# li-kunyi/CUT3R-SLAM

Measured on AMD Instinct MI355X. Metric: frames/sec (ViT pointmap + covisibility-graph tracking step) on 640x480, higher is better.
Workload: dtype f16

## Files before the change

cut3r_slam_amd/_lib.py:

```python
from __future__ import annotations

import ctypes as C
import os

_HERE = os.path.dirname(os.path.abspath(__file__))
LIB_PATH = os.path.join(_HERE, "libcut3r_hip.so")

c_void_p, c_int, c_float, c_ll = C.c_void_p, C.c_int, C.c_float, C.c_longlong


class GemmDesc(C.Structure):
    _fields_ = [
        ("A", c_void_p), ("B", c_void_p), ("C", c_void_p), ("bias", c_void_p), ("res1", c_void_p), ("res2", c_void_p),
        ("M", c_int), ("N", c_int), ("K", c_int), ("lda", c_int), ("ldb", c_int), ("ldc", c_int), ("ldr1", c_int),
        ("ldr2", c_int),
        ("act", c_int), ("out_f16", c_int), ("res1_f16", c_int), ("res2_f16", c_int),
        ("batch", c_int),
        ("strideA", c_ll), ("strideB", c_ll), ("strideC", c_ll), ("strideBias", c_ll), ("strideR1", c_ll),
        ("strideR2", c_ll),
        ("conv_k", c_int), ("H", c_int), ("W", c_int), ("Cin", c_int), ("conv_stride", c_int), ("Ho", c_int),
        ("Wo", c_int), ("relu_in", c_int),
        ("shuf", c_int), ("shuf_cout", c_int), ("shuf_Hin", c_int), ("shuf_Win", c_int),
        ("tile", c_int), ("stages", c_int),
        ("rope_pos", c_void_p), ("rope_table", c_void_p), ("rope_cols", c_int), ("rope_pmin", c_int), ("rope_npos", c_int),
# ... 4 lines not shown


class LcTerm(C.Structure):
    _fields_ = [("a", c_void_p), ("c", c_void_p), ("mask", c_void_p), ("ia", c_int), ("ic", c_int), ("w", c_float), ("pad", c_int)]


SIGNATURES = {
    "cut3r_abi_version": [],
    "cut3r_rope2d": [c_void_p, c_int, c_void_p, c_int, c_int, c_int, c_int, c_ll, c_ll, c_ll, c_float, c_float, c_void_p],
    "cut3r_rope2d_qk": [c_void_p, c_void_p, c_int, c_void_p, c_int, c_int, c_int, c_int, c_ll, c_ll, c_ll, c_ll, c_float, c_float,
                        c_void_p],
    "cut3r_rope2d_tab": [c_void_p, c_void_p, c_ll, c_ll, c_void_p, c_void_p, c_ll, c_ll, c_int, c_int, c_void_p, c_int, c_int, c_float,
                         c_float, c_void_p],
    "cut3r_layernorm": [c_void_p, c_int, c_void_p, c_void_p, c_float, c_int, c_int, c_void_p, c_int, c_void_p, c_int,
                        c_void_p, c_void_p, c_void_p],
    "cut3r_layernorm_dual": [c_void_p, c_int, c_void_p, c_void_p, c_void_p, c_int, c_void_p, c_void_p, c_void_p, c_int, c_float, c_int,
                             c_int, c_void_p],
    "cut3r_gemm_f16": [C.POINTER(GemmDesc), c_void_p],
    "cut3r_gemm_tile_for": [C.POINTER(GemmDesc)],
    "cut3r_gemm_f16_pair": [C.POINTER(GemmDesc), C.POINTER(GemmDesc), c_void_p],
    "cut3r_gemm_kernel_for": [C.POINTER(GemmDesc)],
    "cut3r_gemm_pair_kernel_for": [C.POINTER(GemmDesc), C.POINTER(GemmDesc)],
    "cut3r_gemm_kernel_count": [],
    "cut3r_rope2d_table": [c_void_p, c_int, c_int, c_int, c_float, c_float, c_void_p],
    "cut3r_gemv_f16w": [c_void_p, c_int, c_void_p, c_int, c_void_p, c_void_p, c_int, c_int, c_int, c_int, c_int,
                        c_void_p, c_int, c_int, c_void_p],
    "cut3r_attention_variant": [c_int],
    "cut3r_attention_kernel_for": [c_int, c_int, c_int, c_int],
    "cut3r_attention_f16": [c_void_p, c_void_p, c_void_p, c_void_p, c_int, c_int, c_int, c_int, c_int,
                            c_ll, c_ll, c_ll, c_ll, c_ll, c_ll, c_ll, c_ll, c_float, c_void_p],
    "cut3r_im2col_patch": [c_void_p, c_int, c_int, c_int, c_int, c_int, c_int, c_void_p, c_void_p],
    "cut3r_cast_f32_f16": [c_void_p, c_int, c_void_p, c_int, c_int, c_int, c_void_p],
    "cut3r_colmean": [c_void_p, c_int, c_int, c_int, c_void_p, c_void_p],
    "cut3r_colmean_batched": [c_void_p, c_int, c_ll, c_int, c_int, c_int, c_void_p, c_ll, c_void_p],
    "cut3r_upsample2x_nhwc": [c_void_p, c_void_p, c_int, c_int, c_int, c_int, c_void_p],
    "cut3r_dpt_final": [c_void_p, c_int, c_int, c_void_p, c_void_p, c_int, c_void_p, c_void_p, c_void_p],
    "cut3r_conv3x3_dpt_final": [C.POINTER(GemmDesc), c_void_p, c_void_p, c_int, c_void_p, c_ll, c_void_p, c_ll, c_void_p],
    "cut3r_postprocess_pts": [c_void_p, c_int, c_int, c_int, c_void_p, c_void_p, c_void_p],
    "cut3r_postprocess_pose": [c_void_p, c_int, c_void_p, c_void_p],
    "cut3r_patch_overlap": [c_void_p, c_void_p, c_int, c_int, c_float, c_void_p, c_void_p, c_void_p],
    "cut3r_patch_overlap_chain": [c_void_p, c_void_p, c_int, c_int, c_int, c_float, C.c_double, c_void_p, c_void_p, c_void_p, c_void_p,
                                  c_void_p, c_void_p],
    "cut3r_overlap_fwd": [c_void_p, c_int, C.POINTER(c_float), c_float, c_void_p, c_int, c_float, c_float, c_float, c_float,
                          c_int, c_int, c_int, c_void_p, c_void_p],
    "cut3r_overlap_bwd": [c_void_p, c_int, c_int, c_int, c_int, c_void_p, c_float, c_float, c_float, c_float, c_int, c_int,
                          c_void_p, c_void_p],
# ... 171 lines not shown
```

cut3r_slam_amd/csrc/gemm.hip:

```cpp
#include <cstdlib>
#include "common.h"
#include "dpt_tail.h"
#include "../../include/cut3r_hip.h"

namespace {

constexpr int BK = 64;
constexpr int KCH = BK / 8;

struct GemmArgs {
    const h16* A; const h16* B; void* C;
    const float* bias; const void* res1; const void* res2;
    int M, N, K, lda, ldb, ldc, ldr1, ldr2;
    int act, out_f16, res1_f16, res2_f16;
    long long sA, sB, sC, sBias, sR1, sR2;
    int conv_k, H, W, Cin, cstride, Ho, Wo, relu_in;
    int shuf, shuf_cout, shuf_Hin, shuf_Win;
    int swz;
    int prio;
    const long long* rope_pos; const float* rope_table; int rope_cols, rope_pmin, rope_npos, rope_d;
    const float* ln_stats; const float* ln_c; int ln_nslab; float ln_eps;
    float* stats_out; h16* out16; int ld16;
    const float* dpt_w; const float* dpt_b; float* dpt_pts; float* dpt_conf; long long dpt_pts_vs, dpt_conf_vs;
};
// ... 582 lines not shown
#define CUT3R_TILE_BOUNDS __launch_bounds__(64 * WAVES_M * WAVES_N, (WAVES_M * WAVES_N == 8 && (BM + BN) * BK * 2 * NSTAGE <= 81920) ? 4 : 1)
template <int BM, int BN, int NSTAGE, int WAVES_M = 2, int WAVES_N = 2, int ADDR = 0, int EPI = 0>
__global__ CUT3R_TILE_BOUNDS void gemm_kernel(const GemmArgs g) {
    gemm_tile_body<BM, BN, NSTAGE, WAVES_M, WAVES_N, ADDR, EPI>(g, blockIdx.x, blockIdx.y, blockIdx.z);
}

static int tile_addr_mode(const GemmArgs& g) {
    static const bool off = [] { const char* e = getenv("CUT3R_GEMM_FASTADDR"); return e && atoi(e) == 0; }();
    if (off || (g.K % BK) != 0) return 0;
    if (g.conv_k == 3) return (g.Cin >= 64 && (g.Cin & (g.Cin - 1)) == 0 && g.K == 9 * g.Cin) ? 2 : 0;
    return 1;
}

struct GemmPairArgs { GemmArgs p[2]; int nblk0; };
template <int BM, int BN, int NSTAGE, int WAVES_M = 2, int WAVES_N = 2, int ADDR = 0, int EPI = 0>
__global__ CUT3R_TILE_BOUNDS void gemm_pair_kernel(const GemmPairArgs a) {
    const int sel = (int)blockIdx.x >= a.nblk0 ? 1 : 0;
    gemm_tile_body<BM, BN, NSTAGE, WAVES_M, WAVES_N, ADDR, EPI>(a.p[sel], blockIdx.x - sel * a.nblk0, 0, 0);
}

#ifndef EPI_UNROLL
#define EPI_UNROLL 1
#endif
template <bool CONV3, bool RELU_IN, bool FAST_DMA = false, int EPI = 0, bool LN = false>
DEVINL void gemm256_body(const GemmArgs& g, const int bx, const int bz) {
    constexpr int UNIT = 128 * BK * 2;
    constexpr int BUF = 4 * UNIT;
    static_assert(!LN || EPI == 1 || EPI == 2 || EPI == 6, "the LayerNorm fold feeds the fp16-output epilogues");
    __shared__ __attribute__((aligned(16))) unsigned char smem[2 * BUF + (LN ? 2 * 1024 : 0)];

    const int tid = threadIdx.x, lane = tid & 63, wave = tid >> 6;
    const int wr = wave >> 2, wc = wave & 3;
    const int z = bz;
    const h16* __restrict__ A = g.A + (size_t)z * g.sA;
    const h16* __restrict__ Bm = g.B + (size_t)z * g.sB;
    const int M = g.M, N = g.N, K = g.K;
    int pid_m, pid_n;
    xcd_tile(bx, (M + 255) / 256, (N + 255) / 256, pid_m, pid_n);
    const int m0 = pid_m * 256, n0 = pid_n * 256;
    const h16* zero = reinterpret_cast<const h16*>(g_zero16);

    const int lrow = lane >> 3;
    const int csrc = (lane & 7) ^ lrow;
    const h16* a_ptr[2][2];
    int a_oy[2][2], a_ox[2][2];
    bool a_ok[2][2];
    const h16* b_ptr[2][2];
    bool b_ok[2][2];
#pragma unroll
    for (int q = 0; q < 2; q++)
#pragma unroll
// ... 25 lines not shown
    unsigned a_msk[2][2];
    const int cin_shift = 31 - __builtin_clz((unsigned)(g.Cin > 0 ? g.Cin : 1));
    if (FAST_DMA && CONV3) {
#pragma unroll
        for (int q = 0; q < 2; q++)
#pragma unroll
            for (int i = 0; i < 2; i++) {
                a_pc[q][i] = a_ptr[q][i] + ((ptrdiff_t)a_oy[q][i] * g.W + a_ox[q][i]) * g.Cin + csrc * 8;
                unsigned mk = 0;
#pragma unroll
                for (int t = 0; t < 9; t++) {
                    const int iy = a_oy[q][i] + t / 3, ix = a_ox[q][i] + t % 3;
                    if (a_ok[q][i] && iy >= 0 && iy < g.H && ix >= 0 && ix < g.W) mk |= 1u << t;
                }
                a_msk[q][i] = mk;
            }
    }
#pragma unroll
    for (int q = 0; q < 2; q++)
#pragma unroll
        for (int i = 0; i < 2; i++) {
            const int u = (wave + 8 * i) * 8 + lrow;
            const int gm = min(m0 + (u >> 6) * 128 + q * 64 + (u & 63), M - 1);
            const int gn = min(n0 + (u >> 5) * 64 + q * 32 + (u & 31), N - 1);
            a_off[q][i] = (unsigned)(((size_t)gm * g.lda + csrc * 8) * 2);
            b_off[q][i] = (unsigned)(((size_t)gn * g.ldb + csrc * 8) * 2);
        }
    auto issue_fast = [&](const h16* mat, const unsigned (&off)[2], int kt, int unit) {
        const char* base = reinterpret_cast<const char*>(mat) + (size_t)kt * (BK * 2);
        unsigned char* slot = smem + (kt & 1) * BUF + unit * UNIT;
        const int wave_s = __builtin_amdgcn_readfirstlane(wave);
#pragma unroll
        for (int i = 0; i < 2; i++)
            __builtin_amdgcn_global_load_lds((const __attribute__((address_space(1))) void*)(base + off[i]),
                                             (__attribute__((address_space(3))) void*)(slot + (wave_s + 8 * i) * 1024), 16, 0, 0);
    };
    auto issue_a = [&](int q, int kt, int unit) {
        if (kt >= nt) return;
        if constexpr (fast_dma && !CONV3) { issue_fast(A, a_off[q], kt, unit); return; }
        if constexpr (fast_dma && CONV3) {
            const int k0 = kt * BK;
            const int tap = k0 >> cin_shift;
            const int dy = (tap >= 3) + (tap >= 6), dx = tap - 3 * dy;
            const int delta = (dy * g.W + dx) * g.Cin + (k0 & (g.Cin - 1));
            unsigned char* slot = smem + (kt & 1) * BUF + unit * UNIT;
            const int wave_s = __builtin_amdgcn_readfirstlane(wave);
#pragma unroll
            for (int i = 0; i < 2; i++) {
// ... 148 lines not shown
        CUT3R_QUADRANT(0, 2, fb1);
        CUT3R_BARRIER();
        read_a(buf + 3 * UNIT);
        issue_a(0, t + 2, 0);
        CUT3R_BARRIER();
        CUT3R_QUADRANT(4, 2, fb1);
        CUT3R_BARRIER();
        issue_b(0, t + 2, 1);
        if (t + 2 < nt) wait_vmcnt<4>(); else wait_vmcnt<0>();
        CUT3R_BARRIER();
        CUT3R_QUADRANT(4, 0, fb0);
        CUT3R_BARRIER();
    }
#endif
    if (wr == 0) CUT3R_BARRIER();
#undef CUT3R_QUADRANT

    constexpr int CP = 68;
    float* cs = reinterpret_cast<float*>(smem + wave * 16384);
    const float* bias = g.bias ? g.bias + (size_t)z * g.sBias : nullptr;
    const bool plain = !g.shuf && g.rope_cols == 0;
    const f32x4 zero4 = {0.f, 0.f, 0.f, 0.f};
    const float* lnp = reinterpret_cast<const float*>(smem + 2 * BUF) + wr * 256;
    if constexpr (EPI == 1 || EPI == 2 || EPI == 4 || EPI == 5 || EPI == 6) {
        const int er = lane >> 3, ec = (lane & 7) * 8;
        const int gn = n0 + wc * 64 + ec;
        const bool col_ok = gn + 8 <= N;
        const int gnc = col_ok ? gn : 0;
        const f32x4 b0 = *reinterpret_cast<const f32x4*>(bias + gnc), b1 = *reinterpret_cast<const f32x4*>(bias + gnc + 4);
        f32x4 lc0 = zero4, lc1 = zero4, lpc0 = zero4, lpc1 = zero4;
        if constexpr (LN) { lc0 = *reinterpret_cast<const f32x4*>(g.ln_c + gnc); lc1 = *reinterpret_cast<const f32x4*>(g.ln_c + gnc + 4); }
        const bool rope_here = EPI == 6 && (n0 + wc * 64) < g.rope_cols && col_ok;
        f32x4 pb0 = zero4, pb1 = zero4;
        if (rope_here) {
            const int pc = gnc + ((ec & 16) ? -16 : 16);
            pb0 = *reinterpret_cast<const f32x4*>(bias + pc);
            pb1 = *reinterpret_cast<const f32x4*>(bias + pc + 4);
            if constexpr (LN) { lpc0 = *reinterpret_cast<const f32x4*>(g.ln_c + pc); lpc1 = *reinterpret_cast<const f32x4*>(g.ln_c + pc + 4); }
        }
        constexpr int ROPE_LDS = 48;
        float* tl = cs + 32 * CP;
        int* psl = reinterpret_cast<int*>(tl + ROPE_LDS * 32);
        if (EPI == 6 && __builtin_amdgcn_readfirstlane((n0 + wc * 64) < g.rope_cols)) {
#pragma unroll
            for (int f0 = 0; f0 < ROPE_LDS * 8; f0 += 64) {
                const int f = f0 + lane, p = f >> 3, part = f & 7;
                f32x4 v = zero4;
// ... 696 lines not shown
    g.prio = 0;
    p.k = {gemm_kernel<192, 128, 2, 4, 2, 2, 7>, 512, tile_code(1, 192, 128, 2, 4, 2, 2, 7)};
    p.grid = tile_grid(g.M, g.N, 192, 128, true, 1);
    return CUT3R_OK;
}

extern "C" int cut3r_conv3x3_dpt_final(const cut3r_gemm_desc* d, const float* w, const float* b, int mode, float* pts, long long pts_view_stride,
                                       float* conf, long long conf_view_stride, void* stream) {
    if (!d || mode != 0) return CUT3R_ERR_ARG;
    cut3r_gemm_desc dd = *d;
    dd.C = const_cast<void*>(d->A);
    GemmArgs g;
    Plan<TileFn> p;
    int rc = fill_args(&dd, g);
    if (rc != CUT3R_OK) return rc;
    g.C = nullptr;
    g.dpt_w = w; g.dpt_b = b; g.dpt_pts = pts; g.dpt_conf = conf; g.dpt_pts_vs = pts_view_stride; g.dpt_conf_vs = conf_view_stride;
    rc = plan_dpt_final(&dd, g, p);
    if (rc != CUT3R_OK) return rc;
    hipLaunchKernelGGL(p.k.fn, p.grid, dim3(p.k.block), 0, (hipStream_t)stream, g);
    return cut3r_check_launch();
}

static int select_pair(const cut3r_gemm_desc* d0, const cut3r_gemm_desc* d1, GemmPairArgs& a, Plan<PairFn>& p) {
    if (!d0 || !d1) return CUT3R_ERR_ARG;
    int rc = fill_args(d0, a.p[0]);
    if (rc == CUT3R_OK) rc = fill_args(d1, a.p[1]);
    return rc == CUT3R_OK ? plan_pair(d0, d1, a, p) : rc;
}
extern "C" int cut3r_gemm_pair_kernel_for(const cut3r_gemm_desc* d0, const cut3r_gemm_desc* d1) {
    GemmPairArgs a;
    Plan<PairFn> p;
    return select_pair(d0, d1, a, p) == CUT3R_OK ? p.k.code : 0;
}

extern "C" int cut3r_gemm_f16_pair(const cut3r_gemm_desc* d0, const cut3r_gemm_desc* d1, void* stream) {
    GemmPairArgs a;
    Plan<PairFn> p;
    const int rc = select_pair(d0, d1, a, p);
    if (rc != CUT3R_OK) return rc;
    hipLaunchKernelGGL(p.k.fn, p.grid, dim3(p.k.block), 0, (hipStream_t)stream, a);
    return cut3r_check_launch();
}

extern "C" int cut3r_gemv_f16w(const float* X, int ldx, const void* W, int ldw, const float* bias, float* Y, int ldy, int M,
                               int N, int K, int act, const float* res, int ldr, int silu_in, void* stream) {
// ... 7 lines not shown
```

cut3r_slam_amd/model.py:

```python
from __future__ import annotations

import gc
import math
import os
import re
from dataclasses import dataclass, field
from typing import Dict, List, NamedTuple, Optional

import torch

from . import ops
from .config import Cut3rConfig, production_config, state_dict_schema

F16, F32 = torch.float16, torch.float32


def _env_flag(name: str, default: bool) -> bool:
    return os.environ.get(name, "1" if default else "0") != "0"


def _env_int(name: str, default: int) -> int:
    return int(os.environ.get(name, str(default)))


# ... 61 lines not shown


class Cut3rModel:
    def __init__(self, cfg: Cut3rConfig, state_dict: Dict[str, torch.Tensor], device="cuda:0", minimal: bool = False):
        self.cfg = cfg
        self.device = torch.device(device)
        self.minimal = minimal
        schema = state_dict_schema(cfg)
        missing = [k for k in schema if k not in state_dict]
        if missing:
            raise KeyError(f"state_dict is missing {len(missing)} tensors, e.g. {missing[:4]}")
        for k, shp in schema.items():
            if tuple(state_dict[k].shape) != tuple(shp):
                raise ValueError(f"{k}: shape {tuple(state_dict[k].shape)} != schema {tuple(shp)}")
        self._buf: Dict[tuple, torch.Tensor] = {}
        self._graphs: Dict[tuple, tuple] = {}
        self.use_graphs = _env_flag("CUT3R_GRAPHS", True)
        self.dual_stream = _env_flag("CUT3R_DUAL_STREAM", True)
        self.dual_ln = _env_flag("CUT3R_DUAL_LN", True)
        self.pair_gemm = _env_flag("CUT3R_PAIR_GEMM", False)
        self.pair_rows = _env_int("CUT3R_PAIR_ROWS", 0)
        self.fused_rope = _env_int("CUT3R_FUSED_ROPE", 1)
        self.rope48_rows = _env_int("CUT3R_ROPE48_ROWS", 0)
        self.head_overlap = _env_flag("CUT3R_HEAD_OVERLAP", True)
        self.dpt_fuse = _env_flag("CUT3R_DPT_FUSE", True)
        self.head_chunk = max(1, _env_int("CUT3R_HEAD_CHUNK", 28))
        self.ln_fold = _env_int("CUT3R_LN_FOLD", 1)
        self._head_stream = None
        self._side = None
        self._head_side = None
        self._prep(state_dict)

    @classmethod
    def from_state_dict(cls, cfg, sd, device="cuda:0", **kw):
        return cls(cfg, sd, device, **kw)

    @classmethod
    def from_pretrained(cls, path: str, config: Optional[Cut3rConfig] = None, device="cuda:0", **kw):
        import argparse
        if not os.path.isfile(path):
            raise FileNotFoundError(f"{path}: no checkpoint (this runtime never fetches from a hub)")
        with torch.serialization.safe_globals([argparse.Namespace]):
            ckpt = torch.load(path, map_location="cpu", weights_only=True)
        sd = ckpt["model"] if "model" in ckpt else ckpt
        sd = {(k[7:] if k.startswith("module.") else k): v for k, v in sd.items()}
        if not any(k.startswith("dec_blocks_state") for k in sd):
# ... 125 lines not shown
            c1(q + ".out_conv")
            for u in ("resConfUnit1", "resConfUnit2"):
                c3(f"{q}.{u}.conv1"); c3(f"{q}.{u}.conv2")
        c3(p + ".head.0"); c3(p + ".head.2")
        self.w[p + ".head.4.w"] = sd[p + ".head.4.weight"].reshape(nch, -1).to(device=dev, dtype=F32).contiguous()
        self.w[p + ".head.4.b"] = sd[p + ".head.4.bias"].to(device=dev, dtype=F32).contiguous()

    def buf(self, name, shape, dtype):
        key = (name, tuple(shape), dtype)
        t = self._buf.get(key)
        if t is None:
            t = torch.empty(shape, dtype=dtype, device=self.device)
            self._buf[key] = t
        return t

    def _panel(self, name, rope=None, ln=None):
        L = self.w[name + "@ln"] if ln is not None else self.w[name]
        if rope is not None:
            rope = (rope[0], rope[1], self.cfg.rope_freq, rope[2])
        if ln is not None:
            ln = (ln, L.c, self.cfg.ln_eps)
        return L, rope, ln

    def _linear(self, x16, name, out, act=0, res1=None, res2=None, skinny=False, rope=None, ln=None, emit=None):
        L, rope, ln = self._panel(name, rope, ln)
        return ops.linear(x16, L.w, out, L.b, act, res1, res2, tile=16 if skinny else 0, rope=rope, ln=ln, emit=emit)

    def _project(self, probs, act=0):
        if len(probs) == 1:
            return self._linear(act=act, **probs[0])

        def prob(x16, name, out, res1=None, skinny=False, rope=None, ln=None, emit=None):
            assert not skinny, "the pair kernels have no one-row-per-sequence form"
            L, rope, ln = self._panel(name, rope, ln)
            return (x16, L.w, out, L.b, res1, dict(rope=rope, ln=ln, emit=emit))
        ops.linear_pair(prob(**probs[0]), prob(**probs[1]), act)

    def _folded(self, name):
        return self.ln_fold and (name + "@ln") in self.w

    def _xs(self, tag, x):
        M, Cc = x.shape
        return self.buf(tag + ".x16", (M, Cc), F16), self.buf(tag + ".xst", (Cc // 64, M, 2), F32)

    def _fuse_rope(self, pos, D, rows):
        dims = (64, 48) if (self.fused_rope == 2 or (self.fused_rope and rows <= self.rope48_rows)) else (64,)
        return self.fused_rope and pos is not None and D in dims and pos.is_contiguous() and pos.numel() == 2 * rows

    def _ln(self, x, name, out16=None, out32=None, mod=None):
        g, b = self.w[name]
        ops.layernorm(x, g, b, self.cfg.ln_eps, out16, out32, mod[0] if mod else None, mod[1] if mod else None)

    def _rope(self, t, pos):
        ops.rope_2d_pair(t, pos, None, None, self.cfg.rope_freq, 1.0)

    def _self_attn(self, tag, x_ln16, B, N, heads, pos, p, out, res, ln=None, emit=None):
        Cc = x_ln16.shape[1]
        D = Cc // heads
        sk = N == 1
        qkv = self.buf(tag + ".qkv", (B * N, 3 * Cc), F16)
        fuse = (not sk) and self._fuse_rope(pos, D, B * N)
        self._linear(x_ln16, p + ".qkv", qkv, skinny=sk, rope=(pos, 2 * Cc, D) if fuse else None, ln=ln)
        v5 = qkv.view(B, N, 3, heads, D)
        q, k, v = v5[:, :, 0], v5[:, :, 1], v5[:, :, 2]
        if pos is not None and not fuse:
            ops.rope_2d_pair(q, pos, k, pos, self.cfg.rope_freq, 1.0)
        a = self.buf(tag + ".attn", (B, N, heads, D), F16)
        ops.attention(q, k, v, a, D ** -0.5)
        self._linear(a.view(B * N, Cc), p + ".proj", out, res1=res, skinny=sk, emit=emit)

# ... 94 lines not shown
        s.fold_y = fresh and can(y, Ny, ".cross_attn.projkv")
        s.fold_o = can(out, Nx, ".mlp.fc1")
        s.emit = (out.st, out.x16) if s.fold_o else None
        s.ln16 = self.buf(tag + ".ln16", (B * Nx, C), F16)
        s.y16 = self.buf(tag + ".y16", (B * Ny, C), F16)
        s.qkv = self.buf(tag + ".qkv", (B * Nx, 3 * C), F16)
        s.attn = self.buf(tag + ".attn", (B, Nx, heads, D), F16)
        s.q = self.buf(tag + ".q", (B, Nx, heads, D), F16)
        s.kv = self.buf(tag + ".kv", (B * Ny, 2 * C), F16)
        s.cattn = self.buf(tag + ".cattn", (B, Nx, heads, D), F16)
        s.mlp_h = self.buf(tag + ".mlp_h", (B * Nx, self.w[p + ".mlp.fc1"].npad), F16)
        return s

    def _pair_carries(self, rows):
        return rows <= self.pair_rows

    def _dec_layer(self, blocks, fork=False):
        pair = len(blocks) == 2
        assert not pair or all(s.Nx > 1 and s.Ny > 1 for s in blocks), "pair launches need more than one row per sequence"
        carry = pair and self._pair_carries(max(s.B * max(s.Nx, s.Ny) for s in blocks))
        assert not pair or carry or not any(s.fold_x or s.fold_y or s.fold_o for s in blocks), "the plain pair kernels take no LayerNorm fold"
        fuse = lambda s, pos, n: bool(n > 1 and self._fuse_rope(pos, s.D, s.B * n) and (not pair or (carry and s.D == 64)))
        fuse_x, fuse_y = (lambda s: fuse(s, s.xpos, s.Nx)), (lambda s: fuse(s, s.ypos, s.Ny))

        def each(fn, need=lambda s: True):
            todo = [s for s in blocks if need(s)]
            if fork and len(todo) == 2:
                cur = torch.cuda.current_stream()
                self._side.wait_stream(cur)
                with torch.cuda.stream(self._side):
                    fn(todo[0])
                fn(todo[1])
                cur.wait_stream(self._side)
            else:
                for s in todo:
                    fn(s)

        rows = lambda t: t.view(-1, t.shape[-2] * t.shape[-1])
        skx, sky = (lambda s: s.Nx == 1), (lambda s: s.Ny == 1)
        each(lambda s: self._ln(s.x.x, s.p + ".norm1", out16=s.ln16), lambda s: not (s.fold_x or s.pre_ln))
        self._project([dict(x16=s.x.x16 if s.fold_x else s.ln16, name=s.p + ".attn.qkv", out=s.qkv, skinny=skx(s),
                            rope=(s.xpos, 2 * s.C, s.D) if fuse_x(s) else None, ln=s.x.st if s.fold_x else None) for s in blocks])

        def self_attn(s):
            v5 = s.qkv.view(s.B, s.Nx, 3, s.heads, s.D)
            q, k, v = v5[:, :, 0], v5[:, :, 1], v5[:, :, 2]
            if s.xpos is not None and not fuse_x(s):
                ops.rope_2d_pair(q, s.xpos, k, s.xpos, self.cfg.rope_freq, 1.0)
            ops.attention(q, k, v, s.attn, s.D ** -0.5)
        each(self_attn)
        self._project([dict(x16=rows(s.attn), name=s.p + ".attn.proj", out=s.out.x, res1=s.x.x, skinny=skx(s), emit=s.emit) for s in blocks])
        each(lambda s: self._ln(s.out.x, s.p + ".norm2", out16=s.ln16), lambda s: not s.fold_o)
        self._project([dict(x16=s.out.x16 if s.fold_o else s.ln16, name=s.p + ".cross_attn.projq", out=rows(s.q), skinny=skx(s),
                            rope=(s.xpos, s.C, s.D) if fuse_x(s) else None, ln=s.out.st if s.fold_o else None) for s in blocks])
        rope_q = lambda s: s.xpos is not None and not fuse_x(s)
        norm_y = lambda s: not (s.fold_y or s.pre_ln)

        def q_rope_and_norm_y(s):
            if rope_q(s):
                self._rope(s.q, s.xpos)
            if norm_y(s):
                self._ln(s.y.x, s.p + ".norm_y", out16=s.y16)
        each(q_rope_and_norm_y, lambda s: rope_q(s) or norm_y(s))
        self._project([dict(x16=s.y.x16 if s.fold_y else s.y16, name=s.p + ".cross_attn.projkv", out=s.kv, skinny=sky(s),
                            rope=(s.ypos, s.C, s.D) if fuse_y(s) else None, ln=s.y.st if s.fold_y else None) for s in blocks])

        def cross_attn(s):
            kv4 = s.kv.view(s.B, s.Ny, 2, s.heads, s.D)
            k, v = kv4[:, :, 0], kv4[:, :, 1]
            if s.ypos is not None and not fuse_y(s):
                self._rope(k, s.ypos)
            ops.attention(s.q, k, v, s.cattn, s.D ** -0.5)
        each(cross_attn)
        self._project([dict(x16=rows(s.cattn), name=s.p + ".cross_attn.proj", out=s.out.x, res1=s.out.x, skinny=skx(s), emit=s.emit) for s in blocks])
        each(lambda s: self._ln(s.out.x, s.p + ".norm3", out16=s.ln16), lambda s: not s.fold_o)
        self._project([dict(x16=s.out.x16 if s.fold_o else s.ln16, name=s.p + ".mlp.fc1", out=s.mlp_h, skinny=skx(s),
                            ln=s.out.st if s.fold_o else None) for s in blocks], act=1)
        self._project([dict(x16=s.mlp_h, name=s.p + ".mlp.fc2", out=s.out.x, res1=s.out.x, skinny=skx(s), emit=s.emit) for s in blocks])

    def _dual_norms(self, l, a, s_a):
        pi, ps = f"dec_blocks.{l}", f"dec_blocks_state.{l}"
        Ci = a.shape[1]
        ops.layernorm_dual(a, *self.w[pi + ".norm1"], self.buf("deci.ln16", (a.shape[0], Ci), F16),
                           *self.w[ps + ".norm_y"], self.buf("decs.y16", (a.shape[0], Ci), F16), self.cfg.ln_eps)
        ops.layernorm_dual(s_a, *self.w[ps + ".norm1"], self.buf("decs.ln16", (s_a.shape[0], Ci), F16),
                           *self.w[pi + ".norm_y"], self.buf("deci.y16", (s_a.shape[0], Ci), F16), self.cfg.ln_eps)

    def _mem_inquire(self, gfeat16, mem, B=1):
        cfg = self.cfg
        D = cfg.dec_embed_dim
        x = self.buf("memr.x", (B, 2 * D), F32)
        self._linear(gfeat16, "pose_retriever.proj_q", x[:, :D], skinny=True)
        x[:, D:] = self.masked_token
# ... 407 lines not shown
```

cut3r_slam_amd/ops.py:

```python
from __future__ import annotations

import ctypes as C
import os
from typing import Optional

import torch

from . import _lib, views
from ._lib import GemmDesc, check

F16, F32 = torch.float16, torch.float32


def _stream():
    return C.c_void_p(torch.cuda.current_stream().cuda_stream)


def _p(t: Optional[torch.Tensor]):
    return C.c_void_p(t.data_ptr()) if t is not None else C.c_void_p(0)


def _req(cond, msg):
    if not cond:
        raise ValueError(msg)
# ... 205 lines not shown
    if emit is not None:
        so, o16 = emit
        _cuda(so, o16)
        _req(N % 64 == 0 and so.dtype == F32 and so.is_contiguous() and so.numel() == M * (N // 64) * 2, f"stats_out fp32 [N/64={N // 64}, M={M}, 2]")
        _req(o16.dtype == F16 and o16.shape == (M, N) and o16.stride(1) == 1, "out16 fp16 [M,N]")
        _req(out.dtype == F32 and res1 is not None and res1.dtype == F32 and res2 is None and act == 0 and tile != 16, "emit: fp32 output with an fp32 residual")
        d.stats_out, d.out16, d.ld16 = so.data_ptr(), o16.data_ptr(), o16.stride(0)
    return d


def linear(A, W, out, bias=None, act=0, res1=None, res2=None, tile=0, rope=None, ln=None, emit=None):
    if tile == 16 and A.dim() == 2 and A.shape[0] > 64:
        M = A.shape[0]
        _linear_desc(A, W, out, bias, act, res1, tile, rope, res2=res2)
        for m0 in range(0, M, 64):
            sl = slice(m0, min(M, m0 + 64))
            linear(A[sl], W, out[sl], bias, act, None if res1 is None else res1[sl], None if res2 is None else res2[sl], tile=16)
        return out
    d = _linear_desc(A, W, out, bias, act, res1, tile, rope, ln, emit, res2=res2)
    _launch(d, f"cut3r_gemm_f16 M={d.M} N={d.N} K={d.K}")
    return out


def linear_pair(p0, p1, act=0, tile=0):
    x0 = p0[5] if len(p0) > 5 and p0[5] else {}
    x1 = p1[5] if len(p1) > 5 and p1[5] else {}
    d0 = _linear_desc(p0[0], p0[1], p0[2], p0[3], act, p0[4], tile, pair=True, **x0)
    d1 = _linear_desc(p1[0], p1[1], p1[2], p1[3], act, p1[4], tile, pair=True, **x1)
    _req(d0.N == d1.N and d0.K == d1.K, "pair: same N and K")
    lib = _lib.load()
    check(lib.cut3r_gemm_f16_pair(C.byref(d0), C.byref(d1), _stream()), f"cut3r_gemm_f16_pair M={d0.M}+{d1.M} N={d0.N} K={d0.K}")


def linear_batched(A, W, out, bias=None, act=0, res1=None, tile=0):
    _cuda(A, W, out, bias, res1)
    _req(A.dtype == F16 and W.dtype == F16 and A.dim() == 3 and W.dim() == 3 and out.dim() == 3, "3-D fp16 operands")
    Z, M, K = A.shape
    N = W.shape[1]
    _req(W.shape == (Z, N, K) and out.shape == (Z, M, N), "batched shapes")
    _req(A.stride(2) == 1 and W.stride(2) == 1 and out.stride(2) == 1, "unit inner strides")
    d = GemmDesc()
    _fill_common(d, A, W, out, bias, None, None, act, tile)
    if bias is not None:
        _req(bias.dtype == F32 and bias.shape == (Z, N) and bias.stride(1) == 1, "bias [Z,N]")
        d.strideBias = bias.stride(0)
    if res1 is not None:
# ... 1197 lines not shown
```

include/cut3r_hip.h:

```cpp
#ifndef CUT3R_HIP_H
#define CUT3R_HIP_H
#include <stdint.h>
#ifdef __cplusplus
extern "C" {
#endif

int cut3r_abi_version(void);

int cut3r_rope2d(void* tokens, int dtype, const int64_t* positions, int B, int N, int H, int D,
                 long long sB, long long sN, long long sH, float base, float fwd, void* stream);
int cut3r_rope2d_qk(void* q, void* k, int dtype, const int64_t* positions, int B, int N, int H, int D, long long q_sB,
                    long long q_sN, long long k_sB, long long k_sN, float base, float fwd, void* stream);

int cut3r_rope2d_tab(void* t0, const int64_t* pos0, long long ntok0, long long stride0, void* t1, const int64_t* pos1, long long ntok1,
                     long long stride1, int H, int D, const float* table, int pmin, int npos, float base, float fwd, void* stream);

int cut3r_layernorm(const float* x, int ldx, const float* gamma, const float* beta, float eps, int M, int C,
                    void* y16, int ld16, float* y32, int ld32, const float* mod_scale, const float* mod_shift,
                    void* stream);
int cut3r_layernorm_dual(const float* x, int ldx, const float* g1, const float* b1, void* y1, int ld1, const float* g2,
                         const float* b2, void* y2, int ld2, float eps, int M, int C, void* stream);

typedef struct cut3r_gemm_desc {
    const void* A;
// ... 13 lines not shown
    int shuf;
    int shuf_cout, shuf_Hin, shuf_Win;
    int tile;
    int stages;
    const void* rope_pos;
    const float* rope_table;
    int rope_cols, rope_pmin, rope_npos;
    int rope_d;
    const float* ln_stats;
    const float* ln_colsum;
    int ln_nslab;
    float ln_eps;
    float* stats_out;
    void* out16;
    int ld16;
} cut3r_gemm_desc;
int cut3r_gemm_f16(const cut3r_gemm_desc* d, void* stream);
int cut3r_rope2d_table(float* table, int pmin, int npos, int Q, float base, float fwd, void* stream);
int cut3r_gemm_tile_for(const cut3r_gemm_desc* d);
int cut3r_gemm_f16_pair(const cut3r_gemm_desc* d0, const cut3r_gemm_desc* d1, void* stream);
int cut3r_gemm_kernel_for(const cut3r_gemm_desc* d);
int cut3r_gemm_pair_kernel_for(const cut3r_gemm_desc* d0, const cut3r_gemm_desc* d1);
int cut3r_gemm_kernel_count(void);

int cut3r_gemv_f16w(const float* X, int ldx, const void* W, int ldw, const float* bias, float* Y, int ldy,
                    int M, int N, int K, int act, const float* res, int ldr, int silu_in, void* stream);

int cut3r_attention_f16(const void* q, const void* k, const void* v, void* out, int B, int H, int Nq, int Nk, int D,
                        long long q_sb, long long q_sn, long long k_sb, long long k_sn, long long v_sb, long long v_sn,
                        long long o_sb, long long o_sn, float scale, void* stream);

int cut3r_attention_variant(int v);
int cut3r_attention_kernel_for(int B, int H, int Nq, int D);

int cut3r_im2col_patch(const void* img, int u8, int B, int C, int H, int W, int P, void* out, void* stream);
int cut3r_cast_f32_f16(const float* x, int ldx, void* y, int ldy, int M, int C, void* stream);
int cut3r_colmean(const float* x, int ldx, int M, int C, float* y, void* stream);
int cut3r_colmean_batched(const float* x, int B, long long stride_x, int ldx, int M, int C, float* y, long long stride_y, void* stream);

int cut3r_upsample2x_nhwc(const void* in, void* out, int B, int H, int W, int C, void* stream);
int cut3r_dpt_final(const void* in, int P, int Cin, const float* w, const float* b, int mode, float* pts, float* conf,
                    void* stream);
int cut3r_conv3x3_dpt_final(const cut3r_gemm_desc* d, const float* w, const float* b, int mode, float* pts, long long pts_view_stride,
                            float* conf, long long conf_view_stride, void* stream);
int cut3r_postprocess_pts(const float* raw, int P, int nch, int pos_z, float* pts, float* conf, void* stream);
int cut3r_postprocess_pose(const float* raw, int B, float* out, void* stream);
// ... 277 lines not shown
```

Measured before the change: 5898.

## Fuse 2D RoPE for 48-dim heads into 256-tile GEMM epilogue via column remap

Adds a new 256x256 GEMM epilogue (EPI 8) that applies 2D rotary embedding for head dimension 48 directly on the projection output. It permutes the weight columns so each rotary pair lands in the same 64-column slab, and stages a slice of the cos/sin table plus the token positions in LDS. The model routes qkv, q and kv projections through this path when the existing fused-rope path does not apply, which removes the separate rope kernels and their extra read and write of Q/K. The cost is a more complex epilogue with extra LDS traffic, half-width stores, and a global-memory fallback for positions outside the staged table.

```diff
diff --git a/cut3r_slam_amd/_lib.py b/cut3r_slam_amd/_lib.py
--- a/cut3r_slam_amd/_lib.py
+++ b/cut3r_slam_amd/_lib.py
@@ -50,6 +50,8 @@
     "cut3r_gemm_kernel_for": [C.POINTER(GemmDesc)],
     "cut3r_gemm_pair_kernel_for": [C.POINTER(GemmDesc), C.POINTER(GemmDesc)],
     "cut3r_gemm_kernel_count": [],
+    "cut3r_gemm_rope48_f16": [C.POINTER(GemmDesc), c_void_p],
+    "cut3r_gemm_rope48_col": [c_int, c_int],
     "cut3r_rope2d_table": [c_void_p, c_int, c_int, c_int, c_float, c_float, c_void_p],
     "cut3r_gemv_f16w": [c_void_p, c_int, c_void_p, c_int, c_void_p, c_void_p, c_int, c_int, c_int, c_int, c_int,
                         c_void_p, c_int, c_int, c_void_p],
diff --git a/cut3r_slam_amd/csrc/gemm.hip b/cut3r_slam_amd/csrc/gemm.hip
--- a/cut3r_slam_amd/csrc/gemm.hip
+++ b/cut3r_slam_amd/csrc/gemm.hip
@@ -628,11 +628,17 @@
 #ifndef EPI_UNROLL
 #define EPI_UNROLL 1
 #endif
+__host__ DEVINL int rope48_col(int c) {
+    const int w = c & 63, p = 32 * (c >> 6) + (w & 31);
+    const int h = p / 12, i = p - 12 * h;
+    return 24 * h + i + 12 * (w >> 5);
+}
 template <bool CONV3, bool RELU_IN, bool FAST_DMA = false, int EPI = 0, bool LN = false>
 DEVINL void gemm256_body(const GemmArgs& g, const int bx, const int bz) {
     constexpr int UNIT = 128 * BK * 2;
     constexpr int BUF = 4 * UNIT;
-    static_assert(!LN || EPI == 1 || EPI == 2 || EPI == 6, "the LayerNorm fold feeds the fp16-output epilogues");
+    static_assert(!LN || EPI == 1 || EPI == 2 || EPI == 6 || EPI == 8, "the LayerNorm fold feeds the fp16-output epilogues");
+    static_assert(EPI != 8 || (FAST_DMA && !CONV3 && !RELU_IN), "the column map lives in the fast B addressing of a plain Linear");
     __shared__ __attribute__((aligned(16))) unsigned char smem[2 * BUF + (LN ? 2 * 1024 : 0)];
 
     const int tid = threadIdx.x, lane = tid & 63, wave = tid >> 6;
@@ -704,8 +710,11 @@
         for (int i = 0; i < 2; i++) {
             const int u = (wave + 8 * i) * 8 + lrow;
             const int gm = min(m0 + (u >> 6) * 128 + q * 64 + (u & 63), M - 1);
-            const int gn = min(n0 + (u >> 5) * 64 + q * 32 + (u & 31), N - 1);
-            a_off[q][i] = (unsigned)(((size_t)gm * g.lda + csrc * 8) * 2);
+            int gn = min(n0 + (u >> 5) * 64 + q * 32 + (u & 31), N - 1);
+            if constexpr (EPI == 8) {
+                if (gn < g.rope_cols) gn = rope48_col(gn);
+            }
+            a_off[q][i] =(unsigned)(((size_t)gm * g.lda + csrc * 8) * 2);
             b_off[q][i] = (unsigned)(((size_t)gn * g.ldb + csrc * 8) * 2);
         }
     auto issue_fast = [&](const h16* mat, const unsigned (&off)[2], int kt, int unit) {
@@ -900,7 +909,117 @@
     const bool plain = !g.shuf && g.rope_cols == 0;
     const f32x4 zero4 = {0.f, 0.f, 0.f, 0.f};
     const float* lnp = reinterpret_cast<const float*>(smem + 2 * BUF) + wr * 256;
-    if constexpr (EPI == 1 || EPI == 2 || EPI == 4 || EPI == 5 || EPI == 6) {
+    if constexpr (EPI == 8) {
+        const int er = lane >> 3, ec = (lane & 7) * 8;
+        const int slab = n0 + wc * 64;
+        const bool rope_here = __builtin_amdgcn_readfirstlane(slab < g.rope_cols);
+        const int g0 = rope_here ? rope48_col(slab + ec) : slab + ec;
+        const int g1 = rope_here ? rope48_col(slab + ec + 4) : slab + ec + 4;
+        const f32x4 b0 = *reinterpret_cast<const f32x4*>(bias + g0), b1 = *reinterpret_cast<const f32x4*>(bias + g1);
+        f32x4 lc0 = zero4, lc1 = zero4, lpc0 = zero4, lpc1 = zero4;
+        if constexpr (LN) { lc0 = *reinterpret_cast<const f32x4*>(g.ln_c + g0); lc1 = *reinterpret_cast<const f32x4*>(g.ln_c + g1); }
+        const bool lower = !(ec & 32);
+        const int po = lower ? 12 : -12;
+        f32x4 pb0 = zero4, pb1 = zero4;
+        if (rope_here) {
+            pb0 = *reinterpret_cast<const f32x4*>(bias + g0 + po);
+            pb1 = *reinterpret_cast<const f32x4*>(bias + g1 + po);
+            if constexpr (LN) { lpc0 = *reinterpret_cast<const f32x4*>(g.ln_c + g0 + po); lpc1 = *reinterpret_cast<const f32x4*>(g.ln_c + g1 + po); }
+        }
+        const int x0 = (g0 / 24) & 1, x1 = (g1 / 24) & 1, i0 = g0 % 12, i1 = g1 % 12;
+        constexpr int ROPE_LDS = 48, RQ = 12;
+        float* tl = cs + 32 * CP;
+        int* psl = reinterpret_cast<int*>(tl + ROPE_LDS * 2 * RQ);
+        static_assert((32 * CP + ROPE_LDS * 2 * RQ + 256) * 4 <= 16384, "staging band + table rows + positions in the wave's 16 KiB");
+        if (rope_here) {
+#pragma unroll
+            for (int f0 = 0; f0 < ROPE_LDS * 6; f0 += 64) {
+                const int f = f0 + lane, p = f / 6, part = f - 6 * p;
+                if (f < ROPE_LDS * 6) {
+                    f32x4 v = zero4;
+                    if (p < g.rope_npos) v = *reinterpret_cast<const f32x4*>(g.rope_table + (size_t)(part >= 3) * g.rope_npos * RQ + p * RQ + (part % 3) * 4);
+                    *reinterpret_cast<f32x4*>(tl + p * (2 * RQ) + part * 4) = v;
+                }
+            }
+#pragma unroll
+            for (int i = 0; i < 2; i++) {
+                const int r = lane + 64 * i;
+                const int gmr = min(m0 + wr * 128 + r, M - 1);
+                const longlong2 pp = *reinterpret_cast<const longlong2*>(g.rope_pos + (size_t)gmr * 2);
+                long long py = pp.x - g.rope_pmin, px = pp.y - g.rope_pmin;
+                py = py < 0 ? 0 : (py >= g.rope_npos ? g.rope_npos - 1 : py);
+                px = px < 0 ? 0 : (px >= g.rope_npos ? g.rope_npos - 1 : px);
+                psl[r * 2] = (int)py;
+                psl[r * 2 + 1] = (int)px;
+            }
+            asm volatile("s_waitcnt lgkmcnt(0)" ::: "memory");
+        }
+        h16* crow = (h16*)g.C + (size_t)(m0 + wr * 128 + er) * g.ldc;
+        const size_t step8 = (size_t)8 * g.ldc;
+#pragma unroll
+        for (int mp = 0; mp < 4; mp++) {
+#pragma unroll
+            for (int i = 0; i < 2; i++)
+#pragma unroll
+                for (int j = 0; j < 4; j++)
+#pragma unroll
+                    for (int e = 0; e < 4; e++) cs[(i * 16 + fq * 4 + e) * CP + j * 16 + fr] = acc[mp * 2 + i][j][e];
+            asm volatile("s_waitcnt lgkmcnt(0)" ::: "memory");
+#pragma unroll
+            for (int it = 0; it < 4; it++) {
+                const int rr = it * 8 + er;
+                f32x4 v0 = *reinterpret_cast<const f32x4*>(cs + rr * CP + ec);
+                f32x4 v1 = *reinterpret_cast<const f32x4*>(cs + rr * CP + ec + 4);
+                float rs = 1.f, rm = 0.f;
+                if constexpr (LN) {
+                    const float2 pr = *reinterpret_cast<const float2*>(lnp + 2 * (mp * 32 + rr));
+                    rs = pr.x; rm = pr.y;
+                    v0 = ln_pre4(v0, rs, rm, lc0);
+                    v1 = ln_pre4(v1, rs, rm, lc1);
+                }
+                v0 += b0;
+                v1 += b1;
+                h16* dst = crow + (size_t)(mp * 4 + it) * step8;
+                const bool row_ok = m0 + wr * 128 + mp * 32 + rr < M;
+                if (rope_here) {
+                    f32x4 p0 = *reinterpret_cast<const f32x4*>(cs + rr * CP + (ec ^ 32));
+                    f32x4 p1 = *reinterpret_cast<const f32x4*>(cs + rr * CP + (ec ^ 32) + 4);
+                    if constexpr (LN) { p0 = ln_pre4(p0, rs, rm, lpc0); p1 = ln_pre4(p1, rs, rm, lpc1); }
+                    p0 += pb0;
+                    p1 += pb1;
+                    const int pv0 = psl[(mp * 32 + rr) * 2 + x0], pv1 = psl[(mp * 32 + rr) * 2 + x1];
+                    f32x4 c0, c1, s0, s1;
+                    if (__builtin_amdgcn_ballot_w64(pv0 >= ROPE_LDS || pv1 >= ROPE_LDS) == 0) {
+                        const float* t0 = tl + pv0 * (2 * RQ) + i0;
+                        const float* t1 = tl + pv1 * (2 * RQ) + i1;
+                        c0 = *reinterpret_cast<const f32x4*>(t0); s0 = *reinterpret_cast<const f32x4*>(t0 + RQ);
+                        c1 = *reinterpret_cast<const f32x4*>(t1); s1 = *reinterpret_cast<const f32x4*>(t1 + RQ);
+                    } else {
+                        const float* t0 = g.rope_table + (size_t)pv0 * RQ + i0;
+                        const float* t1 = g.rope_table + (size_t)pv1 * RQ + i1;
+                        c0 = *reinterpret_cast<const f32x4*>(t0); s0 = *reinterpret_cast<const f32x4*>(t0 + (size_t)g.rope_npos * RQ);
+                        c1 = *reinterpret_cast<const f32x4*>(t1); s1 = *reinterpret_cast<const f32x4*>(t1 + (size_t)g.rope_npos * RQ);
+                    }
+#pragma unroll
+                    for (int e = 0; e < 4; e++) {
+                        float t0 = (float)(h16)p0[e] * s0[e], t1 = (float)(h16)p1[e] * s1[e];
+                        asm volatile("" : "+v"(t0), "+v"(t1));
+                        v0[e] = rope_rot((float)(h16)v0[e], c0[e], lower ? -t0 : t0);
+                        v1[e] = rope_rot((float)(h16)v1[e], c1[e], lower ? -t1 : t1);
+                    }
+                    const half4_t o0 = {(h16)v0[0], (h16)v0[1], (h16)v0[2], (h16)v0[3]}, o1 = {(h16)v1[0], (h16)v1[1], (h16)v1[2], (h16)v1[3]};
+                    if (row_ok) {
+                        *reinterpret_cast<half4_t*>(dst + g0) = o0;
+                        *reinterpret_cast<half4_t*>(dst + g1) = o1;
+                    }
+                } else {
+                    const half8_t o = {(h16)v0[0], (h16)v0[1], (h16)v0[2], (h16)v0[3], (h16)v1[0], (h16)v1[1], (h16)v1[2], (h16)v1[3]};
+                    if (row_ok) *reinterpret_cast<half8_t*>(dst + g0) = o;
+                }
+            }
+            asm volatile("s_waitcnt lgkmcnt(0)" ::: "memory");
+        }
+    } else if constexpr (EPI == 1 || EPI == 2 || EPI == 4 || EPI == 5 || EPI == 6) {
         const int er = lane >> 3, ec = (lane & 7) * 8;
         const int gn = n0 + wc * 64 + ec;
         const bool col_ok = gn + 8 <= N;
@@ -1643,6 +1762,37 @@
     return cut3r_check_launch();
 }
 
+static int plan_rope48(const cut3r_gemm_desc* d, GemmArgs& g, Plan<TileFn>& p) {
+    if (d->rope_d != 48 || !d->rope_pos || !d->rope_table || d->rope_npos < 1 || ((uintptr_t)d->rope_table & 15) || ((uintptr_t)d->rope_pos & 15)) return CUT3R_ERR_ARG;
+    if (d->rope_cols <= 0 || d->rope_cols % 192 || d->rope_cols > d->N || (d->N & 255)) return CUT3R_ERR_ARG;
+    if (!d->out_f16 || d->act || d->res1 || d->res2 || d->shuf || d->conv_k == 3 || d->relu_in || batch_of(d) != 1 || d->stats_out) return CUT3R_ERR_ARG;
+    if (!d->bias || ((uintptr_t)d->bias & 15) || (d->ldc & 7)) return CUT3R_ERR_ARG;
+    cut3r_gemm_desc dd = *d;
+    dd.rope_pos = nullptr; dd.rope_table = nullptr; dd.rope_cols = 0; dd.rope_d = 0;
+    if (cut3r_gemm_tile_for(&dd) != 256) return CUT3R_ERR_ARG;
+    const int rc = fill_args(&dd, g);
+    if (rc != CUT3R_OK) return rc;
+    if (!gemm256_fast_ok(g)) return CUT3R_ERR_ARG;
+    g.rope_pos = (const long long*)d->rope_pos; g.rope_table = d->rope_table;
+    g.rope_cols = d->rope_cols; g.rope_pmin = d->rope_pmin; g.rope_npos = d->rope_npos; g.rope_d = 48;
+    const bool ln = g.ln_stats != nullptr;
+    p.k = ln ? Kern<TileFn>{gemm256_kernel<false, false, true, 8, true>, 512u, 300181}
+             : Kern<TileFn>{gemm256_kernel<false, false, true, 8, false>, 512u, 300180};
+    p.grid = tile_grid(g.M, g.N, 256, 256, true, 1);
+    return CUT3R_OK;
+}
+
+extern "C" int cut3r_gemm_rope48_f16(const cut3r_gemm_desc* d, void* stream) {
+    if (!d) return CUT3R_ERR_ARG;
+    GemmArgs g;
+    Plan<TileFn> p;
+    const int rc = plan_rope48(d, g, p);
+    if (rc != CUT3R_OK) return rc;
+    hipLaunchKernelGGL(p.k.fn, p.grid, dim3(p.k.block), 0, (hipStream_t)stream, g);
+    return cut3r_check_launch();
+}
+extern "C" int cut3r_gemm_rope48_col(int c, int rope_cols) { return (c >= 0 && c < rope_cols) ? rope48_col(c) : c; }
+
 static int select_pair(const cut3r_gemm_desc* d0, const cut3r_gemm_desc* d1, GemmPairArgs& a, Plan<PairFn>& p) {
     if (!d0 || !d1) return CUT3R_ERR_ARG;
     int rc = fill_args(d0, a.p[0]);
diff --git a/cut3r_slam_amd/model.py b/cut3r_slam_amd/model.py
--- a/cut3r_slam_amd/model.py
+++ b/cut3r_slam_amd/model.py
@@ -107,6 +107,8 @@
         self.pair_rows = _env_int("CUT3R_PAIR_ROWS", 0)
         self.fused_rope = _env_int("CUT3R_FUSED_ROPE", 1)
         self.rope48_rows = _env_int("CUT3R_ROPE48_ROWS", 0)
+        self.rope48_256 = _env_flag("CUT3R_ROPE48_256", True)
+        self.rope48_force = False
         self.head_overlap = _env_flag("CUT3R_HEAD_OVERLAP", True)
         self.dpt_fuse = _env_flag("CUT3R_DPT_FUSE", True)
         self.head_chunk = max(1, _env_int("CUT3R_HEAD_CHUNK", 28))
@@ -278,16 +280,19 @@
             ln = (ln, L.c, self.cfg.ln_eps)
         return L, rope, ln
 
-    def _linear(self, x16, name, out, act=0, res1=None, res2=None, skinny=False, rope=None, ln=None, emit=None):
+    def _linear(self, x16, name, out, act=0, res1=None, res2=None, skinny=False, rope=None, ln=None, emit=None, rope48=False):
         L, rope, ln = self._panel(name, rope, ln)
+        if rope48:
+            assert not skinny and act == 0 and res1 is None and res2 is None and emit is None
+            return ops.linear_rope48(x16, L.w, out, L.b, rope, ln, tile=256 if self.rope48_force else 0)
         return ops.linear(x16, L.w, out, L.b, act, res1, res2, tile=16 if skinny else 0, rope=rope, ln=ln, emit=emit)
 
     def _project(self, probs, act=0):
         if len(probs) == 1:
             return self._linear(act=act, **probs[0])
 
-        def prob(x16, name, out, res1=None, skinny=False, rope=None, ln=None, emit=None):
-            assert not skinny, "the pair kernels have no one-row-per-sequence form"
+        def prob(x16, name, out, res1=None, skinny=False, rope=None, ln=None, emit=None, rope48=False):
+            assert not skinny and not rope48, "the pair kernels have no one-row-per-sequence form and no column map"
             L, rope, ln = self._panel(name, rope, ln)
             return (x16, L.w, out, L.b, res1, dict(rope=rope, ln=ln, emit=emit))
         ops.linear_pair(prob(**probs[0]), prob(**probs[1]), act)
@@ -302,6 +307,13 @@
     def _fuse_rope(self, pos, D, rows):
         dims = (64, 48) if (self.fused_rope == 2 or (self.fused_rope and rows <= self.rope48_rows)) else (64,)
         return self.fused_rope and pos is not None and D in dims and pos.is_contiguous() and pos.numel() == 2 * rows
+
+    def _rope48_256(self, pos, rows, N, K, cols):
+        if not (self.rope48_256 and self.fused_rope and pos is not None and pos.is_contiguous() and pos.numel() == 2 * rows):
+            return False
+        if self.rope48_force:
+            return N % 256 == 0 and K % 64 == 0 and cols % 192 == 0
+        return ops.linear_rope48_ok(rows, N, K, cols)
 
     def _ln(self, x, name, out16=None, out32=None, mod=None):
         g, b = self.w[name]
@@ -442,6 +454,8 @@
         assert not pair or carry or not any(s.fold_x or s.fold_y or s.fold_o for s in blocks), "the plain pair kernels take no LayerNorm fold"
         fuse = lambda s, pos, n: bool(n > 1 and self._fuse_rope(pos, s.D, s.B * n) and (not pair or (carry and s.D == 64)))
         fuse_x, fuse_y = (lambda s: fuse(s, s.xpos, s.Nx)), (lambda s: fuse(s, s.ypos, s.Ny))
+        r48 = lambda s, pos, n, N, cols: bool(not pair and s.D == 48 and n > 1 and not fuse(s, pos, n) and self._rope48_256(pos, s.B * n, N, s.C, cols))
+        r48_qkv, r48_q, r48_kv = (lambda s: r48(s, s.xpos, s.Nx, 3 * s.C, 2 * s.C)), (lambda s: r48(s, s.xpos, s.Nx, s.C, s.C)), (lambda s: r48(s, s.ypos, s.Ny, 2 * s.C, s.C))
 
         def each(fn, need=lambda s: True):
             todo = [s for s in blocks if need(s)]
@@ -460,20 +474,20 @@
         skx, sky = (lambda s: s.Nx == 1), (lambda s: s.Ny == 1)
         each(lambda s: self._ln(s.x.x, s.p + ".norm1", out16=s.ln16), lambda s: not (s.fold_x or s.pre_ln))
         self._project([dict(x16=s.x.x16 if s.fold_x else s.ln16, name=s.p + ".attn.qkv", out=s.qkv, skinny=skx(s),
-                            rope=(s.xpos, 2 * s.C, s.D) if fuse_x(s) else None, ln=s.x.st if s.fold_x else None) for s in blocks])
+                            rope=(s.xpos, 2 * s.C, s.D) if fuse_x(s) or r48_qkv(s) else None, ln=s.x.st if s.fold_x else None, rope48=r48_qkv(s)) for s in blocks])
 
         def self_attn(s):
             v5 = s.qkv.view(s.B, s.Nx, 3, s.heads, s.D)
             q, k, v = v5[:, :, 0], v5[:, :, 1], v5[:, :, 2]
-            if s.xpos is not None and not fuse_x(s):
+            if s.xpos is not None and not fuse_x(s) and not r48_qkv(s):
                 ops.rope_2d_pair(q, s.xpos, k, s.xpos, self.cfg.rope_freq, 1.0)
             ops.attention(q, k, v, s.attn, s.D ** -0.5)
         each(self_attn)
         self._project([dict(x16=rows(s.attn), name=s.p + ".attn.proj", out=s.out.x, res1=s.x.x, skinny=skx(s), emit=s.emit) for s in blocks])
         each(lambda s: self._ln(s.out.x, s.p + ".norm2", out16=s.ln16), lambda s: not s.fold_o)
         self._project([dict(x16=s.out.x16 if s.fold_o else s.ln16, name=s.p + ".cross_attn.projq", out=rows(s.q), skinny=skx(s),
-                            rope=(s.xpos, s.C, s.D) if fuse_x(s) else None, ln=s.out.st if s.fold_o else None) for s in blocks])
-        rope_q = lambda s: s.xpos is not None and not fuse_x(s)
+                            rope=(s.xpos, s.C, s.D) if fuse_x(s) or r48_q(s) else None, ln=s.out.st if s.fold_o else None, rope48=r48_q(s)) for s in blocks])
+        rope_q = lambda s: s.xpos is not None and not fuse_x(s) and not r48_q(s)
         norm_y = lambda s: not (s.fold_y or s.pre_ln)
 
         def q_rope_and_norm_y(s):
@@ -483,12 +497,12 @@
                 self._ln(s.y.x, s.p + ".norm_y", out16=s.y16)
         each(q_rope_and_norm_y, lambda s: rope_q(s) or norm_y(s))
         self._project([dict(x16=s.y.x16 if s.fold_y else s.y16, name=s.p + ".cross_attn.projkv", out=s.kv, skinny=sky(s),
-                            rope=(s.ypos, s.C, s.D) if fuse_y(s) else None, ln=s.y.st if s.fold_y else None) for s in blocks])
+                            rope=(s.ypos, s.C, s.D) if fuse_y(s) or r48_kv(s) else None, ln=s.y.st if s.fold_y else None, rope48=r48_kv(s)) for s in blocks])
 
         def cross_attn(s):
             kv4 = s.kv.view(s.B, s.Ny, 2, s.heads, s.D)
             k, v = kv4[:, :, 0], kv4[:, :, 1]
-            if s.ypos is not None and not fuse_y(s):
+            if s.ypos is not None and not fuse_y(s) and not r48_kv(s):
                 self._rope(k, s.ypos)
             ops.attention(s.q, k, v, s.cattn, s.D ** -0.5)
         each(cross_attn)
diff --git a/cut3r_slam_amd/ops.py b/cut3r_slam_amd/ops.py
--- a/cut3r_slam_amd/ops.py
+++ b/cut3r_slam_amd/ops.py
@@ -251,6 +251,21 @@
     return out
 
 
+def linear_rope48_ok(M, N, K, cols):
+    if N % 256 or K % 64 or cols <= 0 or cols % 192 or cols > N:
+        return False
+    d = GemmDesc()
+    d.M, d.N, d.K, d.batch, d.out_f16 = M, N, K, 1, 1
+    return _lib.load().cut3r_gemm_tile_for(C.byref(d)) == 256
+
+
+def linear_rope48(A, W, out, bias, rope, ln=None, tile=0):
+    _req(rope is not None and len(rope) > 3 and rope[3] == 48 and bias is not None, "linear_rope48: heads of 48 and a bias")
+    d = _linear_desc(A, W, out, bias, 0, None, tile, rope, ln)
+    check(_lib.load().cut3r_gemm_rope48_f16(C.byref(d), _stream()), f"cut3r_gemm_rope48_f16 M={d.M} N={d.N} K={d.K} cols={d.rope_cols}")
+    return out
+
+
 def linear_pair(p0, p1, act=0, tile=0):
     x0 = p0[5] if len(p0) > 5 and p0[5] else {}
     x1 = p1[5] if len(p1) > 5 and p1[5] else {}
diff --git a/include/cut3r_hip.h b/include/cut3r_hip.h
--- a/include/cut3r_hip.h
+++ b/include/cut3r_hip.h
@@ -59,6 +59,8 @@
 int cut3r_gemm_kernel_for(const cut3r_gemm_desc* d);
 int cut3r_gemm_pair_kernel_for(const cut3r_gemm_desc* d0, const cut3r_gemm_desc* d1);
 int cut3r_gemm_kernel_count(void);
+int cut3r_gemm_rope48_f16(const cut3r_gemm_desc* d, void* stream);
+int cut3r_gemm_rope48_col(int c, int rope_cols);
 
 int cut3r_gemv_f16w(const float* X, int ldx, const void* W, int ldw, const float* bias, float* Y, int ldy,
                     int M, int N, int K, int act, const float* res, int ldr, int silu_in, void* stream);
```

After: 5953, median of 6. No clear change (+0.9%).
